# larrybb626/diffusion_models_dsdiff

Measured on AMD Instinct MI355X. Metric: 256x256 cDDPM slices/sec (1000-step), higher is better.
Workload: dtype f32 (operands split exactly into 3 bf16 pieces, 6 bf16-MFMA products, f32 accumulate)

## Files before the change

diffusion_models_dsdiff_amd/csrc/conv.hip:

```cpp
#include "device_common.h"

#include <string>

#include <cstdlib>

namespace dsd {

static constexpr size_t DIRECT_LDS_MAX = 128 * 1024;
static constexpr int BM = 128;
static constexpr int BK = 32;
static constexpr int LDS_STRIDE = 36;

struct ConvP {
    const float* x;
    const float* w;
    const float* bias;
    const float* emb;
    const float* res;
    float* y;
    int64_t x_bs;
    int N, H, W, Cin, Cout, OH, OW, ks, stride, pad, ups, emb_stride, out_nchw;
    int M, Ktot, cchunks, IHg, IWg, tiles_m, tiles_n, ohw;
    unsigned x_bytes, w_bytes;
    int y_ld;
// ... 215 lines not shown
    const int nwg = gridDim.x;
    int L = blockIdx.x;
    {
        const int cpx = nwg >> 3;
        if (L < (cpx << 3)) L = (L & 7) * cpx + (L >> 3);
    }
    const int tile_n = L % p.tiles_n;
    const int tile_m = L / p.tiles_n;
    const int m0 = tile_m * BM;
    const int n0 = tile_n * (NT * 32);

    const int col4 = tid & 7;
    const int srow = tid >> 3;
    int a_h[4], a_w[4];
    unsigned a_nb[4];
    bool a_ok[4];
#pragma unroll
    for (int i = 0; i < 4; ++i) {
        int m = m0 + srow + 32 * i;
        a_ok[i] = m < p.M;
        m = a_ok[i] ? m : 0;
        const int n = m / p.ohw;
        const int r = m - n * p.ohw;
        const int oh = r / p.OW;
        const int ow = r - oh * p.OW;
        a_h[i] = oh * p.stride - p.pad;
        a_w[i] = ow * p.stride - p.pad;
        a_nb[i] = (unsigned)n * (unsigned)p.x_bs + (unsigned)(col4 * 4);
    }
    unsigned b_voff[NT];
#pragma unroll
    for (int j = 0; j < NT; ++j) {
        const int n = n0 + srow + 32 * j;
        b_voff[j] = n < p.Cout ? ((unsigned)n * (unsigned)p.Ktot + (unsigned)(col4 * 4)) * 4u : OOB;
    }
    unsigned a_voff[4];
    auto tap_offsets = [&](int kh, int kw) {
#pragma unroll
        for (int i = 0; i < 4; ++i) {
            int ih = a_h[i] + kh, iw = a_w[i] + kw;
            const bool ok = a_ok[i] && (unsigned)ih < (unsigned)p.IHg && (unsigned)iw < (unsigned)p.IWg;
            if (p.ups) {
                ih >>= 1;
                iw >>= 1;
            }
            a_voff[i] = ok ? (a_nb[i] + (unsigned)(ih * p.W + iw) * (unsigned)p.Cin) * 4u : OOB;
        }
    };
    f32x4 ra[4], rb[NT];
    auto load_tile = [&](int soff_a, int soff_b) {
#pragma unroll
        for (int i = 0; i < 4; ++i) ra[i] = __builtin_bit_cast(f32x4, __builtin_amdgcn_raw_buffer_load_b128(rx, a_voff[i], soff_a, 0));
#pragma unroll
        for (int j = 0; j < NT; ++j) rb[j] = __builtin_bit_cast(f32x4, __builtin_amdgcn_raw_buffer_load_b128(rw, b_voff[j], soff_b, 0));
    };

    f32x16 acc[NT];
#pragma unroll
    for (int j = 0; j < NT; ++j)
#pragma unroll
        for (int r = 0; r < 16; ++r) acc[j][r] = 0.f;

    const int lrow = lane & 31;
    const int half = lane >> 5;
    const float* a_frag = As + (wave * 32 + lrow) * LDS_STRIDE + 4 * half;
    const float* b_frag = Bs + lrow * LDS_STRIDE + 4 * half;
    float* a_st = As + srow * LDS_STRIDE + col4 * 4;
    float* b_st = Bs + srow * LDS_STRIDE + col4 * 4;

    const int KT = p.ks * p.ks * p.cchunks;
    int kh = 0, kw = 0, cc = 0, tap = 0;
    tap_offsets(0, 0);
    load_tile(0, 0);
    for (int kt = 0; kt < KT; ++kt) {
        __syncthreads();
#pragma unroll
        for (int i = 0; i < 4; ++i) *reinterpret_cast<f32x4*>(a_st + 32 * i * LDS_STRIDE) = ra[i];
#pragma unroll
        for (int j = 0; j < NT; ++j) *reinterpret_cast<f32x4*>(b_st + 32 * j * LDS_STRIDE) = rb[j];
        __syncthreads();
        if (kt + 1 < KT) {
            if (++cc == p.cchunks) {
                cc = 0;
                ++tap;
                if (++kw == p.ks) {
                    kw = 0;
                    ++kh;
                }
                tap_offsets(kh, kw);
            }
            load_tile(cc * (BK * 4), (tap * p.Cin + cc * BK) * 4);
        }
        conv_tile_mfma<NT, 4, LDS_STRIDE>(a_frag, b_frag, acc);
    }
    conv_epilogue<NT>(p, acc, m0, n0, wave, lrow, half);
}

__global__ __launch_bounds__(256) void conv_direct_lds_kernel(ConvP p) {
    extern __shared__ float wl[];
    const int tid = threadIdx.x;
    for (int i = tid; i < p.Ktot * p.Cout; i += 256) {
        const int k = i / p.Cout, co = i - k * p.Cout;
        wl[i] = p.w[(int64_t)co * p.Ktot + k];
    }
    __syncthreads();
    const int c4n = p.Cout >> 2;
    const int PIX = 64;
    const int64_t pix0 = (int64_t)blockIdx.x * PIX;
    for (int idx = tid; idx < PIX * c4n; idx += 256) {
        const int pl = idx / c4n, c4 = idx - pl * c4n;
        const int64_t m = pix0 + pl;
        if (m >= p.M) break;
        const int nb = (int)(m / p.ohw);
        const int r = (int)(m - (int64_t)nb * p.ohw);
        const int oh = r / p.OW, ow = r - oh * p.OW;
        float4 acc = make_float4(0.f, 0.f, 0.f, 0.f);
        int k = 0;
        for (int kh = 0; kh < p.ks; ++kh)
            for (int kw = 0; kw < p.ks; ++kw) {
                int ih = oh * p.stride - p.pad + kh, iw = ow * p.stride - p.pad + kw;
                const bool ok = (unsigned)ih < (unsigned)p.IHg && (unsigned)iw < (unsigned)p.IWg;
                if (p.ups) {
                    ih >>= 1;
                    iw >>= 1;
                }
                const float* src = p.x + (int64_t)nb * p.x_bs + ((int64_t)ih * p.W + iw) * p.Cin;
                for (int ci = 0; ci < p.Cin; ++ci, ++k) {
                    const float xv = ok ? src[ci] : 0.f;
                    const float4 w4 = *reinterpret_cast<const float4*>(wl + k * p.Cout + c4 * 4);
                    acc.x = fmaf(xv, w4.x, acc.x);
                    acc.y = fmaf(xv, w4.y, acc.y);
                    acc.z = fmaf(xv, w4.z, acc.z);
                    acc.w = fmaf(xv, w4.w, acc.w);
                }
            }
        float v[4] = {acc.x, acc.y, acc.z, acc.w};
#pragma unroll
        for (int q = 0; q < 4; ++q) {
            const int n = c4 * 4 + q;
            if (p.bias) v[q] += p.bias[n];
            if (p.emb) v[q] += p.emb[(int64_t)nb * p.emb_stride + n];
            if (p.res) v[q] += p.res[m * p.Cout + n];
        }
        if (p.out_nchw) {
            for (int q = 0; q < 4; ++q) p.y[((int64_t)nb * p.Cout + c4 * 4 + q) * p.ohw + r] = v[q];
        } else {
            *reinterpret_cast<float4*>(p.y + m * p.y_ld + c4 * 4) = make_float4(v[0], v[1], v[2], v[3]);
        }
    }
}

template <int KMAX, bool STATS>
__global__ __launch_bounds__(256) void conv_direct_cols_kernel(ConvP p, int W4, int ppb, double* __restrict__ stats, int chunks) {
    __shared__ double sm[STATS ? 1024 : 1][2];
    const int rpi = blockDim.x / W4;
    const int row = threadIdx.x / W4;
    const int c4 = threadIdx.x - row * W4;
    double ss[4] = {0.0, 0.0, 0.0, 0.0}, qq[4] = {0.0, 0.0, 0.0, 0.0};
    float4 w[KMAX];
#pragma unroll
    for (int k = 0; k < KMAX; ++k) {
        if (k < p.Ktot) {
            w[k].x = p.w[(int64_t)(c4 * 4 + 0) * p.Ktot + k];
            w[k].y = p.w[(int64_t)(c4 * 4 + 1) * p.Ktot + k];
            w[k].z = p.w[(int64_t)(c4 * 4 + 2) * p.Ktot + k];
            w[k].w = p.w[(int64_t)(c4 * 4 + 3) * p.Ktot + k];
        } else {
            w[k] = make_float4(0.f, 0.f, 0.f, 0.f);
        }
    }
    int dh[KMAX], dw[KMAX], dc[KMAX];
#pragma unroll
    for (int k = 0; k < KMAX; ++k) {
        const int tap = k / p.Cin;
        dc[k] = k - tap * p.Cin;
        dh[k] = tap / p.ks - p.pad;
        dw[k] = tap - (tap / p.ks) * p.ks - p.pad;
    }
    const float4 b4 = p.bias ? *reinterpret_cast<const float4*>(p.bias + c4 * 4) : make_float4(0.f, 0.f, 0.f, 0.f);
    const int64_t m_end = min((int64_t)p.M, ((int64_t)blockIdx.x + 1) * ppb);
    int64_t m = (int64_t)blockIdx.x * ppb + row;
    int nb = (int)(m / p.ohw);
    int oh = (int)(m - (int64_t)nb * p.ohw) / p.OW;
    int ow = (int)(m - (int64_t)nb * p.ohw) - oh * p.OW;
    for (; m < m_end; m += rpi, ow += rpi) {
        while (ow >= p.OW) {
            ow -= p.OW;
            if (++oh == p.OH) {
                oh = 0;
                ++nb;
            }
        }
        float4 acc = make_float4(0.f, 0.f, 0.f, 0.f);
        const float* xb = p.x + (int64_t)nb * p.x_bs;
#pragma unroll
        for (int k = 0; k < KMAX; ++k) {
            int ih = oh * p.stride + dh[k], iw = ow * p.stride + dw[k];
            const bool ok = (k < p.Ktot) & ((unsigned)ih < (unsigned)p.IHg) & ((unsigned)iw < (unsigned)p.IWg);
            ih >>= p.ups;
            iw >>= p.ups;
            const float xv = ok ? xb[((int64_t)ih * p.W + iw) * p.Cin + dc[k]] : 0.f;
            acc.x = fmaf(xv, w[k].x, acc.x);
            acc.y = fmaf(xv, w[k].y, acc.y);
            acc.z = fmaf(xv, w[k].z, acc.z);
            acc.w = fmaf(xv, w[k].w, acc.w);
        }
        acc.x += b4.x; acc.y += b4.y; acc.z += b4.z; acc.w += b4.w;
        if (p.emb) {
            const float4 e = *reinterpret_cast<const float4*>(p.emb + (int64_t)nb * p.emb_stride + c4 * 4);
            acc.x += e.x; acc.y += e.y; acc.z += e.z; acc.w += e.w;
        }
        if (p.res) {
            const float4 e = *reinterpret_cast<const float4*>(p.res + m * p.Cout + c4 * 4);
            acc.x += e.x; acc.y += e.y; acc.z += e.z; acc.w += e.w;
        }
        *reinterpret_cast<float4*>(p.y + m * p.y_ld + c4 * 4) = acc;
        if (STATS) {
            const double a = acc.x, b = acc.y, c = acc.z, d = acc.w;
            ss[0] += a; qq[0] = fma(a, a, qq[0]);
            ss[1] += b; qq[1] = fma(b, b, qq[1]);
            ss[2] += c; qq[2] = fma(c, c, qq[2]);
            ss[3] += d; qq[3] = fma(d, d, qq[3]);
        }
    }
    if (STATS) {
        if (row > 0) {
#pragma unroll
            for (int e = 0; e < 4; ++e) {
                sm[row * p.Cout + c4 * 4 + e][0] = ss[e];
                sm[row * p.Cout + c4 * 4 + e][1] = qq[e];
            }
        }
        __syncthreads();
        if (row == 0) {
            for (int r = 1; r < rpi; ++r)
#pragma unroll
                for (int e = 0; e < 4; ++e) {
                    ss[e] += sm[r * p.Cout + c4 * 4 + e][0];
                    qq[e] += sm[r * p.Cout + c4 * 4 + e][1];
                }
            const int64_t m0 = (int64_t)blockIdx.x * ppb;
            const int n0 = (int)(m0 / p.ohw), chunk = (int)((m0 - (int64_t)n0 * p.ohw) / ppb);
            double* o = stats + (((int64_t)n0 * chunks + chunk) * p.Cout + c4 * 4) * 2;
#pragma unroll
            for (int e = 0; e < 4; ++e) {
                o[2 * e] = ss[e];
                o[2 * e + 1] = qq[e];
            }
        }
    }
}

__global__ __launch_bounds__(256) void conv_scalar_kernel(ConvP p) {
    const int64_t total = (int64_t)p.M * p.Cout;
    for (int64_t i = (int64_t)blockIdx.x * 256 + threadIdx.x; i < total; i += (int64_t)gridDim.x * 256) {
        const int64_t m = i / p.Cout;
        const int n = (int)(i - m * p.Cout);
        const int nb = (int)(m / p.ohw);
        const int r = (int)(m - (int64_t)nb * p.ohw);
        const int oh = r / p.OW, ow = r - oh * p.OW;
        float acc = 0.f;
        const float* wr = p.w + (int64_t)n * p.Ktot;
        for (int kh = 0; kh < p.ks; ++kh)
            for (int kw = 0; kw < p.ks; ++kw) {
                int ih = oh * p.stride - p.pad + kh, iw = ow * p.stride - p.pad + kw;
                if (!((unsigned)ih < (unsigned)p.IHg && (unsigned)iw < (unsigned)p.IWg)) continue;
                if (p.ups) {
                    ih >>= 1;
                    iw >>= 1;
                }
                const float* src = p.x + (int64_t)nb * p.x_bs + ((int64_t)ih * p.W + iw) * p.Cin;
                const float* wk = wr + (kh * p.ks + kw) * p.Cin;
                for (int ci = 0; ci < p.Cin; ++ci) acc = fmaf(src[ci], wk[ci], acc);
            }
        if (p.bias) acc += p.bias[n];
        if (p.emb) acc += p.emb[(int64_t)nb * p.emb_stride + n];
        if (p.res) acc += p.res[m * p.Cout + n];
        if (p.out_nchw)
            p.y[((int64_t)nb * p.Cout + n) * p.ohw + r] = acc;
        else
            p.y[m * p.y_ld + n] = acc;
    }
}

__global__ void pack_ohwi_kernel(const float* __restrict__ src, float* __restrict__ dst, int Cout, int Cin, int kk) {
    const int64_t total = (int64_t)Cout * Cin * kk;
    for (int64_t i = (int64_t)blockIdx.x * blockDim.x + threadIdx.x; i < total; i += (int64_t)gridDim.x * blockDim.x) {
        const int ci = (int)(i % Cin);
        const int64_t r = i / Cin;
        const int t = (int)(r % kk);
        const int co = (int)(r / kk);
        dst[i] = src[((int64_t)co * Cin + ci) * kk + t];
    }
}

void pack_ohwi(const float* w_oihw, float* w_ohwi, int Cout, int Cin, int ks, hipStream_t s) {
    const int64_t total = (int64_t)Cout * Cin * ks * ks;
    const int blocks = (int)std::min<int64_t>((total + 255) / 256, 65535);
    hipLaunchKernelGGL(pack_ohwi_kernel, dim3(blocks), dim3(256), 0, s, w_oihw, w_ohwi, Cout, Cin, ks * ks);
    check_launch("pack_ohwi");
}

double conv2d_flops(const ConvArgs& a) {
    int OH, OW;
    conv_out_hw(a, &OH, &OW);
    return 2.0 * a.N * OH * OW * (double)a.Cout * a.ks * a.ks * a.Cin;
}

double conv2d_exec_flops(const ConvArgs& a) { return a.w_subpixel ? conv2d_flops(a) * 4.0 / 9.0 : conv2d_flops(a); }

static int conv_variant(const ConvArgs& a) {
    if (a.variant >= 0) return a.variant;
    static const int env = [] {
        const char* e = getenv("DSD_CONV_VARIANT");
        return e ? atoi(e) : 0;
    }();
    return env;
}

static int pick_nt(int Cout, int tiles_m, int precision, int lanes = 1) {
    static const int force = [] {
        const char* e = getenv("DSD_FORCE_NT");
        return e ? atoi(e) : 0;
    }();
    if (force >= 1 && force <= 5) return force;
    const int t32 = cdiv(Cout, 32);
    const double t_fix = precision == PREC_F32 ? 500.0 : 700.0;
    const double t_mf = precision == PREC_F32 ? 1024.0 : (precision == PREC_BF16X6 ? 384.0 : 192.0);
    int best = 1;
    double best_t = 1e300;
    for (int nt = 5; nt >= 1; --nt) {
        const int64_t blocks = (int64_t)tiles_m * cdiv(t32, nt) * std::max(1, lanes);
        const double t = (double)cdiv(blocks, 512) * (t_fix + nt * t_mf);
        if (t < best_t * 0.999) {
            best_t = t;
            best = nt;
        }
    }
    return best;
}

static int direct_cols_ppb(const ConvArgs& a, int64_t M, int ohw, bool with_stats) {
    const int W4 = a.Cout / 4, rpi = 256 / W4;
    if (!with_stats) return std::max(rpi * 8, cdiv(cdiv(M, 8192), rpi) * rpi);
    for (int ppb = 128; ppb >= 16; ppb >>= 1)
        if (ohw % ppb == 0) return ppb;
    return 0;
}

ConvRoute conv2d_route(const ConvArgs& a, bool replan) {
    ConvRoute r;
    conv_out_hw(a, &r.OH, &r.OW);
    r.M = (int64_t)a.N * r.OH * r.OW;
    const int ohw = r.OH * r.OW, Ktot = a.ks * a.ks * a.Cin;
    r.precision = a.precision == PREC_F32 || !conv2d_split_eligible(a) ? PREC_F32 : a.precision;
    r.nt = pick_nt(a.Cout, cdiv(r.M, BM), r.precision, a.lanes);
    if (a.w_subpixel) {
        r.family = CONV_SUBPIXEL;
        r.precision = PREC_BF16X6;
        r.nt = 5;
        r.structure = 2;
        r.tap_reuse = true;
        r.stats_chunks = conv2d_subpixel_shape_ok(a) ? 4 * a.H * a.W / (2 * BM) : 0;
        return r;
    }
    if (a.Cin % 4 != 0 || Ktot < 32) {
        if (a.Cout % 4 == 0 && a.Cout / 4 <= 256 && Ktot <= 9 && !a.out_nchw && (!a.emb || a.emb_stride % 4 == 0)) {
            r.family = CONV_DIRECT_COLS;
            const int ppb = direct_cols_ppb(a, r.M, ohw, true);
            r.stats_chunks = ppb ? ohw / ppb : 0;
        } else {
            r.family = a.Cout % 4 == 0 && (size_t)Ktot * a.Cout * sizeof(float) <= DIRECT_LDS_MAX ? CONV_DIRECT_LDS : CONV_SCALAR;
        }
        return r;
    }
    if (r.precision == PREC_BF16X6 && conv2d_wino_eligible(a)) {
        r.family = CONV_WINO;
        r.stats_chunks = conv2d_wino_stats_chunks(a);
        return r;
    }
    if (r.precision == PREC_F32) {
        const int64_t x_bs = a.x_bs >= 0 ? a.x_bs : (int64_t)a.H * a.W * a.Cin;
        const int64_t xb = ((int64_t)(a.N - 1) * x_bs + (int64_t)a.H * a.W * a.Cin) * 4, wb = (int64_t)a.Cout * Ktot * 4;
        r.family = a.Cin % BK == 0 && xb < 0xFFFFFF00ll && wb < 0xFFFFFF00ll && conv_variant(a) == 0 ? CONV_MFMA_BUF : CONV_MFMA;
        return r;
    }
    r.family = CONV_SPLIT;
    int nt_p, ks_p, ad_p, nt_d, ks_d, ad_d;
    conv2d_split_plan(a, r.nt, &nt_p, &ks_p, &ad_p, true);
    conv2d_split_plan(a, r.nt, &nt_d, &ks_d, &ad_d, false);
    r.nt = replan ? nt_p : nt_d;
    r.ksplit = replan ? ks_p : ks_d;
    r.structure = replan ? ad_p : ad_d;
    r.launches = r.ksplit > 1 ? 2 : 1;
    r.scratch_bytes = r.ksplit > 1 ? (size_t)r.ksplit * r.M * a.Cout * sizeof(float) : 0;
// ... 99 lines not shown
```

diffusion_models_dsdiff_amd/csrc/norm.hip:

```cpp
#include "device_common.h"

#include <cstdlib>

namespace dsd {

static constexpr int GN_GROUPS = 32;

struct GnGeom {
    int threads;
    int k;
    int rpi;
    int ppc;
    int nchunk;
};

static GnGeom gn_geom(int HW, int C) {
    GnGeom g{};
    const int cols = C / 4;
    if (cols <= 256) {
        g.k = 1;
        g.rpi = 256 / cols;
        g.threads = g.rpi * cols;
    } else {
        g.k = 2;
        while (cols % g.k != 0 || cols / g.k > 256) ++g.k;
        g.rpi = 1;
        g.threads = cols / g.k;
    }
    int ppc = cdiv(HW, 256);
    if (ppc < 32) ppc = 32;
    ppc = cdiv(ppc, g.rpi) * g.rpi;
    g.ppc = ppc;
    g.nchunk = cdiv(HW, ppc);
    return g;
}

int gn_nchunks(int HW, int C) { return gn_geom(HW, C).nchunk; }

template <int K>
__global__ __launch_bounds__(256) void gn_stats_kernel(const float* __restrict__ x, int HW, int C, int rpi, int ppc,
                                                       double* __restrict__ partial) {
    extern __shared__ double sm[];
    const int cols = C >> 2;
    const int colsk = cols / K;
    const int tid = threadIdx.x;
    const int row = tid / colsk;
    const int col0 = tid - row * colsk;
    const int n = blockIdx.y, chunk = blockIdx.x;
    const int p0 = chunk * ppc;
    const int p1 = min(HW, p0 + ppc);
    double s[K][4], q[K][4];
#pragma unroll
    for (int k = 0; k < K; ++k)
#pragma unroll
        for (int e = 0; e < 4; ++e) s[k][e] = q[k][e] = 0.0;
    const float* base = x + (int64_t)n * HW * C;
    auto accum = [&](int k, const float4 v) {
        const double a = v.x, b = v.y, c = v.z, d = v.w;
        s[k][0] += a; q[k][0] = fma(a, a, q[k][0]);
        s[k][1] += b; q[k][1] = fma(b, b, q[k][1]);
        s[k][2] += c; q[k][2] = fma(c, c, q[k][2]);
        s[k][3] += d; q[k][3] = fma(d, d, q[k][3]);
    };
    int p = p0 + row;
    for (; p + 3 * rpi < p1; p += 4 * rpi) {
        float4 v[4][K];
#pragma unroll
        for (int u = 0; u < 4; ++u)
#pragma unroll
            for (int k = 0; k < K; ++k)
                v[u][k] = reinterpret_cast<const float4*>(base + (int64_t)(p + u * rpi) * C)[col0 + k * colsk];
#pragma unroll
        for (int u = 0; u < 4; ++u)
#pragma unroll
            for (int k = 0; k < K; ++k) accum(k, v[u][k]);
    }
    for (; p < p1; p += rpi) {
        const float4* rp = reinterpret_cast<const float4*>(base + (int64_t)p * C);
#pragma unroll
        for (int k = 0; k < K; ++k) accum(k, rp[col0 + k * colsk]);
    }
#pragma unroll
    for (int k = 0; k < K; ++k)
#pragma unroll
        for (int e = 0; e < 4; ++e) {
            const int c = (col0 + k * colsk) * 4 + e;
            sm[((int64_t)row * C + c) * 2 + 0] = s[k][e];
            sm[((int64_t)row * C + c) * 2 + 1] = q[k][e];
        }
    __syncthreads();
    for (int c = tid; c < C; c += blockDim.x) {
        double ss = 0.0, qq = 0.0;
        for (int r = 0; r < rpi; ++r) {
            ss += sm[((int64_t)r * C + c) * 2 + 0];
            qq += sm[((int64_t)r * C + c) * 2 + 1];
        }
        double* o = partial + (((int64_t)n * gridDim.x + chunk) * C + c) * 2;
        o[0] = ss;
        o[1] = qq;
    }
}

void gn_stats(const float* x, int N, int HW, int C, double* partial, int nchunk, hipStream_t s) {
    DSD_CHECK(C % GN_GROUPS == 0 && C % 4 == 0, "GroupNorm32: C=%d must be a multiple of 32", C);
    const GnGeom g = gn_geom(HW, C);
    DSD_CHECK(g.nchunk == nchunk, "gn_stats: chunk count mismatch");
    const size_t lds = (size_t)g.rpi * C * 2 * sizeof(double);
    DSD_CHECK(lds <= 64 * 1024, "gn_stats: C=%d too large", C);
    const dim3 grid(g.nchunk, N), block(g.threads);
    switch (g.k) {
        case 1: hipLaunchKernelGGL(gn_stats_kernel<1>, grid, block, lds, s, x, HW, C, g.rpi, g.ppc, partial); break;
        case 2: hipLaunchKernelGGL(gn_stats_kernel<2>, grid, block, lds, s, x, HW, C, g.rpi, g.ppc, partial); break;
        case 3: hipLaunchKernelGGL(gn_stats_kernel<3>, grid, block, lds, s, x, HW, C, g.rpi, g.ppc, partial); break;
        case 4: hipLaunchKernelGGL(gn_stats_kernel<4>, grid, block, lds, s, x, HW, C, g.rpi, g.ppc, partial); break;
        default: fail("gn_stats: C=%d needs %d columns per thread (unsupported)", C, g.k);
    }
    check_launch("gn_stats");
}

__global__ __launch_bounds__(256) void gn_finalize_kernel(GnSrc s0, GnSrc s1, int HW, int C,
                                                          const float* __restrict__ gamma,
                                                          const float* __restrict__ beta, float eps,
                                                          const float* __restrict__ film, int film_stride,
                                                          float* __restrict__ scale, float* __restrict__ shift) {
    __shared__ double red[256][2];
    __shared__ float mean_s, rstd_s;
    const int g = blockIdx.x, n = blockIdx.y, tid = threadIdx.x;
    const int cpg = C / GN_GROUPS;
    const int g0 = g * cpg, g1 = g0 + cpg;
    double ss = 0.0, qq = 0.0;
#pragma unroll
    for (int k = 0; k < 2; ++k) {
        const GnSrc& sr = k == 0 ? s0 : s1;
        if (!sr.p) continue;
        const int lo = max(g0, sr.c0), hi = min(g1, sr.c0 + sr.c);
        const int ncol = hi - lo;
        if (ncol <= 0) continue;
        const int items = sr.chunks * ncol;
        const double* base = sr.p + (int64_t)n * sr.chunks * sr.c * 2;
        for (int it = tid; it < items; it += 256) {
            const int ch = it / ncol, c = lo + (it - ch * ncol) - sr.c0;
            const double* o = base + ((int64_t)ch * sr.c + c) * 2;
            ss += o[0];
            qq += o[1];
        }
    }
    red[tid][0] = ss;
    red[tid][1] = qq;
    __syncthreads();
    for (int st = 128; st > 0; st >>= 1) {
        if (tid < st) {
            red[tid][0] += red[tid + st][0];
            red[tid][1] += red[tid + st][1];
        }
        __syncthreads();
    }
    if (tid == 0) {
        const double cnt = (double)HW * cpg;
        const double mean = red[0][0] / cnt;
        double var = red[0][1] / cnt - mean * mean;
        if (var < 0.0) var = 0.0;
        mean_s = (float)mean;
        rstd_s = (float)(1.0 / sqrt(var + (double)eps));
    }
    __syncthreads();
    for (int c = g0 + tid; c < g1; c += 256) {
        float sc = rstd_s * gamma[c];
        float sh = beta[c] - mean_s * sc;
        if (film) {
            const float f = 1.f + film[(int64_t)n * film_stride + c];
            sc *= f;
            sh = sh * f + film[(int64_t)n * film_stride + C + c];
        }
        scale[(int64_t)n * C + c] = sc;
        shift[(int64_t)n * C + c] = sh;
    }
}

void gn_finalize(const GnSrc& s0, const GnSrc& s1, int N, int HW, int C, const float* gamma, const float* beta,
                 float eps, const float* film, int film_stride, float* scale, float* shift, hipStream_t s) {
    DSD_CHECK(s0.p && s0.c0 == 0 && s0.c + (s1.p ? s1.c : 0) == C && (!s1.p || s1.c0 == s0.c),
              "gn_finalize: the statistic sources do not cover the %d channels", C);
    if (N == 0) return;
    hipLaunchKernelGGL(gn_finalize_kernel, dim3(GN_GROUPS, N), dim3(256), 0, s, s0, s1, HW, C, gamma, beta, eps, film,
                       film_stride, scale, shift);
    check_launch("gn_finalize");
}

template <int ACT, int V>
__global__ __launch_bounds__(256) void gn_small_kernel(const float* __restrict__ x, int HW, int C, const float* __restrict__ gamma,
                                                       const float* __restrict__ beta, float eps, const float* __restrict__ film,
                                                       int film_stride, float* __restrict__ y) {
    constexpr int U = 8;
    __shared__ double red[4][2];
    __shared__ float mean_s, rstd_s;
    const int g = blockIdx.x, n = blockIdx.y, tid = threadIdx.x, lane = tid & 63, wave = tid >> 6;
    const int cpg = C / GN_GROUPS, cv = cpg / V;
    const float* xb = x + (int64_t)n * HW * C + g * cpg;
    float* yb = y + (int64_t)n * HW * C + g * cpg;
    const int items = HW * cv;
    auto off = [&](int i) {
        const int p = i / cv, c = i - p * cv;
        return (int64_t)p * C + c * V;
    };
    double s = 0.0, q = 0.0;
    for (int i0 = tid; i0 < items; i0 += 256 * U) {
        float v[U][V];
#pragma unroll
        for (int u = 0; u < U; ++u) {
            const int i = i0 + u * 256;
#pragma unroll
            for (int k = 0; k < V; ++k) v[u][k] = 0.f;
            if (i < items) {
                if (V == 2) {
                    const float2 t = *reinterpret_cast<const float2*>(xb + off(i));
                    v[u][0] = t.x;
                    v[u][V - 1] = t.y;
                } else {
                    v[u][0] = xb[off(i)];
                }
            }
        }
#pragma unroll
        for (int u = 0; u < U; ++u)
#pragma unroll
            for (int k = 0; k < V; ++k) {
                const double d = v[u][k];
                s += d;
                q = fma(d, d, q);
            }
    }
    for (int o = 32; o > 0; o >>= 1) {
        s += __shfl_xor(s, o);
        q += __shfl_xor(q, o);
    }
    if (lane == 0) {
        red[wave][0] = s;
        red[wave][1] = q;
    }
    __syncthreads();
    if (tid == 0) {
        const double a = (red[0][0] + red[1][0]) + (red[2][0] + red[3][0]);
        const double b = (red[0][1] + red[1][1]) + (red[2][1] + red[3][1]);
        const double cnt = (double)HW * cpg;
        const double mean = a / cnt;
        double var = b / cnt - mean * mean;
        if (var < 0.0) var = 0.0;
        mean_s = (float)mean;
        rstd_s = (float)(1.0 / sqrt(var + (double)eps));
    }
    __syncthreads();
    const float mean = mean_s, rstd = rstd_s;
    auto coef = [&](int ch, float& sc, float& sh) {
        sc = rstd * gamma[ch];
        sh = beta[ch] - mean * sc;
        if (film) {
            const float f = 1.f + film[(int64_t)n * film_stride + ch];
            sc *= f;
            sh = sh * f + film[(int64_t)n * film_stride + C + ch];
        }
    };
    for (int i0 = tid; i0 < items; i0 += 256 * U) {
        float v[U][V];
#pragma unroll
        for (int u = 0; u < U; ++u) {
            const int i = i0 + u * 256;
            if (i < items) {
                if (V == 2) {
                    const float2 t = *reinterpret_cast<const float2*>(xb + off(i));
                    v[u][0] = t.x;
                    v[u][V - 1] = t.y;
                } else {
                    v[u][0] = xb[off(i)];
                }
            }
        }
#pragma unroll
        for (int u = 0; u < U; ++u) {
            const int i = i0 + u * 256;
            if (i >= items) continue;
            const int p = i / cv, c = (i - p * cv) * V;
            float o[V];
#pragma unroll
            for (int k = 0; k < V; ++k) {
                float sc, sh;
                coef(g * cpg + c + k, sc, sh);
                o[k] = fmaf(v[u][k], sc, sh);
                if (ACT == ACT_SILU) o[k] = silu_f(o[k]);
            }
            if (V == 2)
                *reinterpret_cast<float2*>(yb + (int64_t)p * C + c) = make_float2(o[0], o[V - 1]);
            else
                yb[(int64_t)p * C + c] = o[0];
        }
    }
}

bool gn_small_ok(int HW, int C) {
    static const bool on = getenv("DSD_GN_SMALL") != nullptr;
    return on && C % GN_GROUPS == 0 && (int64_t)HW * (C / GN_GROUPS) <= 32768;
}

void gn_small(const float* x, int N, int HW, int C, const float* gamma, const float* beta, float eps, const float* film,
              int film_stride, int act, float* y, hipStream_t s) {
    if ((int64_t)N * HW * C == 0) return;
    const bool v2 = (C / GN_GROUPS) % 2 == 0;
    const dim3 grid(GN_GROUPS, N), block(256);
#define DSD_GNS(A, VV) hipLaunchKernelGGL((gn_small_kernel<A, VV>), grid, block, 0, s, x, HW, C, gamma, beta, eps, film, film_stride, y)
    if (act == ACT_SILU) {
        if (v2) DSD_GNS(ACT_SILU, 2); else DSD_GNS(ACT_SILU, 1);
    } else {
        if (v2) DSD_GNS(ACT_NONE, 2); else DSD_GNS(ACT_NONE, 1);
    }
#undef DSD_GNS
    check_launch("gn_small");
}

template <int K, int ACT>
__global__ __launch_bounds__(256) void avg_stats_kernel(const float4* __restrict__ a, const float4* __restrict__ b,
                                                        const float4* __restrict__ c, const float4* __restrict__ d,
                                                        float div, int HW, int C, int rpi, int ppc, float* __restrict__ dst,
                                                        int dstC, int coff, int bmask, double* __restrict__ partial) {
    extern __shared__ double sm[];
    const int cols = C >> 2;
    const int colsk = cols / K;
    const int tid = threadIdx.x;
    const int row = tid / colsk;
    const int col0 = tid - row * colsk;
    const int n = blockIdx.y, chunk = blockIdx.x;
    const int p0 = chunk * ppc;
    const int p1 = min(HW, p0 + ppc);
    double s[K][4], q[K][4];
#pragma unroll
    for (int k = 0; k < K; ++k)
#pragma unroll
        for (int e = 0; e < 4; ++e) s[k][e] = q[k][e] = 0.0;
    const int64_t sb = (int64_t)n * HW * cols;
    for (int p = p0 + row; p < p1; p += rpi) {
#pragma unroll
        for (int k = 0; k < K; ++k) {
            const int c4 = col0 + k * colsk;
            const int64_t is = (int64_t)p * cols + c4, i = sb + is;
            float4 v = a[(bmask & 1) ? is : i];
            if (b) { const float4 t = b[(bmask & 2) ? is : i]; v.x += t.x; v.y += t.y; v.z += t.z; v.w += t.w; }
            if (c) { const float4 t = c[(bmask & 4) ? is : i]; v.x += t.x; v.y += t.y; v.z += t.z; v.w += t.w; }
            if (d) { const float4 t = d[(bmask & 8) ? is : i]; v.x += t.x; v.y += t.y; v.z += t.z; v.w += t.w; }
            if (div != 1.f) { v.x /= div; v.y /= div; v.z /= div; v.w /= div; }
            if (ACT == ACT_SILU) { v.x = silu_f(v.x); v.y = silu_f(v.y); v.z = silu_f(v.z); v.w = silu_f(v.w); }
            *reinterpret_cast<float4*>(dst + ((int64_t)n * HW + p) * dstC + coff + c4 * 4) = v;
            const double x0 = v.x, x1 = v.y, x2 = v.z, x3 = v.w;
            s[k][0] += x0; q[k][0] = fma(x0, x0, q[k][0]);
            s[k][1] += x1; q[k][1] = fma(x1, x1, q[k][1]);
            s[k][2] += x2; q[k][2] = fma(x2, x2, q[k][2]);
            s[k][3] += x3; q[k][3] = fma(x3, x3, q[k][3]);
        }
    }
#pragma unroll
    for (int k = 0; k < K; ++k)
#pragma unroll
        for (int e = 0; e < 4; ++e) {
            const int cc = (col0 + k * colsk) * 4 + e;
            sm[((int64_t)row * C + cc) * 2 + 0] = s[k][e];
            sm[((int64_t)row * C + cc) * 2 + 1] = q[k][e];
        }
    __syncthreads();
    for (int cc = tid; cc < C; cc += blockDim.x) {
        double ss = 0.0, qq = 0.0;
        for (int r = 0; r < rpi; ++r) {
            ss += sm[((int64_t)r * C + cc) * 2 + 0];
            qq += sm[((int64_t)r * C + cc) * 2 + 1];
        }
        double* o = partial + (((int64_t)n * gridDim.x + chunk) * C + cc) * 2;
        o[0] = ss;
        o[1] = qq;
    }
}

void avg_into_stats(const float* a, const float* b, const float* c, const float* d, float div, int N, int HW, int C,
                    float* dst, int dstC, int coff, int act, int bmask, double* partial, int nchunk, hipStream_t s) {
    DSD_CHECK(C % 4 == 0 && dstC % 4 == 0 && coff % 4 == 0, "avg_into_stats: channel counts must be multiples of 4");
    if ((int64_t)N * HW * C == 0) return;
    const GnGeom g = gn_geom(HW, C);
    DSD_CHECK(g.nchunk == nchunk, "avg_into_stats: chunk count mismatch");
    const size_t lds = (size_t)g.rpi * C * 2 * sizeof(double);
    DSD_CHECK(lds <= 64 * 1024, "avg_into_stats: C=%d too large", C);
    const dim3 grid(g.nchunk, N), block(g.threads);
#define DSD_AVG(KK)                                                                                                          \
    if (act == ACT_SILU)                                                                                                     \
        hipLaunchKernelGGL((avg_stats_kernel<KK, ACT_SILU>), grid, block, lds, s, (const float4*)a, (const float4*)b,        \
                           (const float4*)c, (const float4*)d, div, HW, C, g.rpi, g.ppc, dst, dstC, coff, bmask, partial);  \
    else                                                                                                                     \
        hipLaunchKernelGGL((avg_stats_kernel<KK, ACT_NONE>), grid, block, lds, s, (const float4*)a, (const float4*)b,        \
                           (const float4*)c, (const float4*)d, div, HW, C, g.rpi, g.ppc, dst, dstC, coff, bmask, partial);
    switch (g.k) {
        case 1: DSD_AVG(1) break;
        case 2: DSD_AVG(2) break;
        case 3: DSD_AVG(3) break;
        case 4: DSD_AVG(4) break;
        default: fail("avg_into_stats: C=%d needs %d columns per thread (unsupported)", C, g.k);
    }
#undef DSD_AVG
    check_launch("avg_into_stats");
}


template <int ACT>
__global__ __launch_bounds__(256) void affine_act_kernel(const float4* __restrict__ x, int HW, int cols, int W, int ppc,
                                                         const float4* __restrict__ scale, const float4* __restrict__ shift,
                                                         float4* __restrict__ y) {
    const int n = blockIdx.y;
    const int rpi = blockDim.x / W;
    const int row = threadIdx.x / W;
    const int cw = threadIdx.x - row * W;
    const int p0 = blockIdx.x * ppc;
    const int p1 = min(HW, p0 + ppc);
    const float4* xs = x + (int64_t)n * HW * cols;
    float4* ys = y + (int64_t)n * HW * cols;
    auto act = [](float4 v, const float4 sc, const float4 sh) {
        float4 o;
        o.x = fmaf(v.x, sc.x, sh.x);
        o.y = fmaf(v.y, sc.y, sh.y);
        o.z = fmaf(v.z, sc.z, sh.z);
        o.w = fmaf(v.w, sc.w, sh.w);
        if (ACT == ACT_SILU) {
            o.x = silu_f(o.x);
            o.y = silu_f(o.y);
            o.z = silu_f(o.z);
            o.w = silu_f(o.w);
        }
        return o;
    };
    for (int c4 = cw; c4 < cols; c4 += W) {
        const float4 sc = scale[(int64_t)n * cols + c4];
        const float4 sh = shift[(int64_t)n * cols + c4];
        int p = p0 + row;
        for (; p + 3 * rpi < p1; p += 4 * rpi) {
            const int64_t i0 = (int64_t)p * cols + c4, st = (int64_t)rpi * cols;
            const float4 v0 = xs[i0], v1 = xs[i0 + st], v2 = xs[i0 + 2 * st], v3 = xs[i0 + 3 * st];
            ys[i0] = act(v0, sc, sh);
            ys[i0 + st] = act(v1, sc, sh);
            ys[i0 + 2 * st] = act(v2, sc, sh);
            ys[i0 + 3 * st] = act(v3, sc, sh);
        }
        for (; p < p1; p += rpi) {
            const int64_t i0 = (int64_t)p * cols + c4;
            ys[i0] = act(xs[i0], sc, sh);
        }
    }
}

void affine_act(const float* x, int N, int HW, int C, const float* scale, const float* shift, int act, float* y,
                hipStream_t s) {
    const int cols = C / 4;
    if ((int64_t)N * HW * cols == 0) return;
    const int W = std::min(cols, 256);
    const int rpi = 256 / W, threads = rpi * W;
    int nchunk = std::max(1, std::min(4096 / std::max(N, 1), HW / (4 * rpi)));
    const int ppc = cdiv(cdiv(HW, nchunk), rpi) * rpi;
    nchunk = cdiv(HW, ppc);
    const dim3 grid((unsigned)nchunk, (unsigned)N);
    if (act == ACT_SILU)
        hipLaunchKernelGGL(affine_act_kernel<ACT_SILU>, grid, dim3(threads), 0, s, (const float4*)x, HW, cols, W, ppc,
                           (const float4*)scale, (const float4*)shift, (float4*)y);
    else
        hipLaunchKernelGGL(affine_act_kernel<ACT_NONE>, grid, dim3(threads), 0, s, (const float4*)x, HW, cols, W, ppc,
                           (const float4*)scale, (const float4*)shift, (float4*)y);
    check_launch("affine_act");
}

__global__ __launch_bounds__(256) void layer_norm_kernel(const float* __restrict__ x, int64_t rows, int C,
                                                         const float* __restrict__ gamma,
                                                         const float* __restrict__ beta, float eps,
                                                         float* __restrict__ y) {
    const int lane = threadIdx.x & 63;
    const int64_t row = (int64_t)blockIdx.x * 4 + (threadIdx.x >> 6);
    if (row >= rows) return;
    const float* xr = x + row * C;
    float s = 0.f;
    for (int c = lane; c < C; c += 64) s += xr[c];
    for (int o = 32; o > 0; o >>= 1) s += __shfl_xor(s, o);
    const float mean = s / C;
    float q = 0.f;
    for (int c = lane; c < C; c += 64) {
        const float d = xr[c] - mean;
        q = fmaf(d, d, q);
    }
    for (int o = 32; o > 0; o >>= 1) q += __shfl_xor(q, o);
    const float rstd = 1.f / sqrtf(q / C + eps);
    for (int c = lane; c < C; c += 64) y[row * C + c] = (xr[c] - mean) * rstd * gamma[c] + beta[c];
}

void layer_norm(const float* x, int64_t rows, int C, const float* gamma, const float* beta, float eps, float* y,
                hipStream_t s) {
    if (rows == 0) return;
    hipLaunchKernelGGL(layer_norm_kernel, dim3(cdiv(rows, 4)), dim3(256), 0, s, x, rows, C, gamma, beta, eps, y);
    check_launch("layer_norm");
}

}
```

Baseline: 0.04022.

## Stage conv inputs in LDS, vectorize GN stat reads, unroll avg-stats loads

The direct small-K conv kernel now has each thread gather one output pixel's input patch into shared memory, so the im2col gather happens once per pixel instead of once per output column group. All column threads then reuse the staged values, and the embedding load is cached per batch index. The stats scratch arrays move to a planar layout to cut LDS bank conflicts. GroupNorm finalize now reads partial sums as double2 with 4-way unrolling and reduces with wave shuffles instead of an LDS tree. avg_stats_kernel unrolls loads across pixels and sources and multiplies by an exact power-of-two reciprocal instead of dividing. These kernels are small or bandwidth-bound, the extra syncthreads and LDS use may lower occupancy, and the overall effect on a 1000-step run dominated by MFMA convs is likely small.

```diff
diff --git a/diffusion_models_dsdiff_amd/csrc/conv.hip b/diffusion_models_dsdiff_amd/csrc/conv.hip
--- a/diffusion_models_dsdiff_amd/csrc/conv.hip
+++ b/diffusion_models_dsdiff_amd/csrc/conv.hip
@@ -391,7 +391,9 @@
 
 template <int KMAX, bool STATS>
 __global__ __launch_bounds__(256) void conv_direct_cols_kernel(ConvP p, int W4, int ppb, double* __restrict__ stats, int chunks) {
-    __shared__ double sm[STATS ? 1024 : 1][2];
+    constexpr int XV = (KMAX + 1 + 3) / 4;
+    __shared__ uint4 xs[256 * XV];
+    __shared__ double sm[STATS ? 2048 : 1];
     const int rpi = blockDim.x / W4;
     const int row = threadIdx.x / W4;
     const int c4 = threadIdx.x - row * W4;
@@ -408,66 +410,88 @@
             w[k] = make_float4(0.f, 0.f, 0.f, 0.f);
         }
     }
-    int dh[KMAX], dw[KMAX], dc[KMAX];
-#pragma unroll
-    for (int k = 0; k < KMAX; ++k) {
-        const int tap = k / p.Cin;
-        dc[k] = k - tap * p.Cin;
-        dh[k] = tap / p.ks - p.pad;
-        dw[k] = tap - (tap / p.ks) * p.ks - p.pad;
-    }
     const float4 b4 = p.bias ? *reinterpret_cast<const float4*>(p.bias + c4 * 4) : make_float4(0.f, 0.f, 0.f, 0.f);
-    const int64_t m_end = min((int64_t)p.M, ((int64_t)blockIdx.x + 1) * ppb);
-    int64_t m = (int64_t)blockIdx.x * ppb + row;
-    int nb = (int)(m / p.ohw);
-    int oh = (int)(m - (int64_t)nb * p.ohw) / p.OW;
-    int ow = (int)(m - (int64_t)nb * p.ohw) - oh * p.OW;
-    for (; m < m_end; m += rpi, ow += rpi) {
-        while (ow >= p.OW) {
-            ow -= p.OW;
-            if (++oh == p.OH) {
-                oh = 0;
-                ++nb;
-            }
-        }
-        float4 acc = make_float4(0.f, 0.f, 0.f, 0.f);
-        const float* xb = p.x + (int64_t)nb * p.x_bs;
-#pragma unroll
-        for (int k = 0; k < KMAX; ++k) {
-            int ih = oh * p.stride + dh[k], iw = ow * p.stride + dw[k];
-            const bool ok = (k < p.Ktot) & ((unsigned)ih < (unsigned)p.IHg) & ((unsigned)iw < (unsigned)p.IWg);
-            ih >>= p.ups;
-            iw >>= p.ups;
-            const float xv = ok ? xb[((int64_t)ih * p.W + iw) * p.Cin + dc[k]] : 0.f;
-            acc.x = fmaf(xv, w[k].x, acc.x);
-            acc.y = fmaf(xv, w[k].y, acc.y);
-            acc.z = fmaf(xv, w[k].z, acc.z);
-            acc.w = fmaf(xv, w[k].w, acc.w);
-        }
-        acc.x += b4.x; acc.y += b4.y; acc.z += b4.z; acc.w += b4.w;
-        if (p.emb) {
-            const float4 e = *reinterpret_cast<const float4*>(p.emb + (int64_t)nb * p.emb_stride + c4 * 4);
-            acc.x += e.x; acc.y += e.y; acc.z += e.z; acc.w += e.w;
-        }
-        if (p.res) {
-            const float4 e = *reinterpret_cast<const float4*>(p.res + m * p.Cout + c4 * 4);
-            acc.x += e.x; acc.y += e.y; acc.z += e.z; acc.w += e.w;
-        }
-        *reinterpret_cast<float4*>(p.y + m * p.y_ld + c4 * 4) = acc;
-        if (STATS) {
-            const double a = acc.x, b = acc.y, c = acc.z, d = acc.w;
-            ss[0] += a; qq[0] = fma(a, a, qq[0]);
-            ss[1] += b; qq[1] = fma(b, b, qq[1]);
-            ss[2] += c; qq[2] = fma(c, c, qq[2]);
-            ss[3] += d; qq[3] = fma(d, d, qq[3]);
+    const int64_t m_begin = (int64_t)blockIdx.x * ppb;
+    const int64_t m_end = min((int64_t)p.M, m_begin + ppb);
+    const int T = blockDim.x;
+    float4 e4 = make_float4(0.f, 0.f, 0.f, 0.f);
+    int nb_e = -1;
+    for (int64_t mt = m_begin; mt < m_end; mt += T) {
+        const int tn = (int)min((int64_t)T, m_end - mt);
+        if (mt != m_begin) __syncthreads();
+        if (const int pl = threadIdx.x; pl < tn) {
+            const int m = (int)(mt + pl);
+            const int nb = m / p.ohw;
+            const int r = m - nb * p.ohw;
+            const int oh = r / p.OW, ow = r - oh * p.OW;
+            const float* xb = p.x + (int64_t)nb * p.x_bs;
+            unsigned t[XV * 4];
+#pragma unroll
+            for (int k = 0; k < XV * 4; ++k) t[k] = 0u;
+#pragma unroll
+            for (int k = 0; k < KMAX; ++k) {
+                if (k >= p.Ktot) break;
+                const int tap = k / p.Cin;
+                const int kh = tap / p.ks;
+                int ih = oh * p.stride + kh - p.pad, iw = ow * p.stride + (tap - kh * p.ks) - p.pad;
+                const bool ok = ((unsigned)ih < (unsigned)p.IHg) & ((unsigned)iw < (unsigned)p.IWg);
+                ih >>= p.ups;
+                iw >>= p.ups;
+                const float xv = ok ? xb[((int64_t)ih * p.W + iw) * p.Cin + (k - tap * p.Cin)] : 0.f;
+                t[k] = __float_as_uint(xv);
+            }
+            t[KMAX] = (unsigned)nb;
+#pragma unroll
+            for (int i = 0; i < XV; ++i) xs[pl * XV + i] = make_uint4(t[4 * i], t[4 * i + 1], t[4 * i + 2], t[4 * i + 3]);
+        }
+        __syncthreads();
+        for (int pl = row; pl < tn; pl += rpi) {
+            const int64_t m = mt + pl;
+            unsigned t[XV * 4];
+#pragma unroll
+            for (int i = 0; i < XV; ++i) {
+                const uint4 v = xs[pl * XV + i];
+                t[4 * i] = v.x; t[4 * i + 1] = v.y; t[4 * i + 2] = v.z; t[4 * i + 3] = v.w;
+            }
+            float4 acc = make_float4(0.f, 0.f, 0.f, 0.f);
+#pragma unroll
+            for (int k = 0; k < KMAX; ++k) {
+                const float xv = __uint_as_float(t[k]);
+                acc.x = fmaf(xv, w[k].x, acc.x);
+                acc.y = fmaf(xv, w[k].y, acc.y);
+                acc.z = fmaf(xv, w[k].z, acc.z);
+                acc.w = fmaf(xv, w[k].w, acc.w);
+            }
+            acc.x += b4.x; acc.y += b4.y; acc.z += b4.z; acc.w += b4.w;
+            if (p.emb) {
+                const int nb = (int)t[KMAX];
+                if (nb != nb_e) {
+                    e4 = *reinterpret_cast<const float4*>(p.emb + (int64_t)nb * p.emb_stride + c4 * 4);
+                    nb_e = nb;
+                }
+                acc.x += e4.x; acc.y += e4.y; acc.z += e4.z; acc.w += e4.w;
+            }
+            if (p.res) {
+                const float4 e = *reinterpret_cast<const float4*>(p.res + m * p.Cout + c4 * 4);
+                acc.x += e.x; acc.y += e.y; acc.z += e.z; acc.w += e.w;
+            }
+            *reinterpret_cast<float4*>(p.y + m * p.y_ld + c4 * 4) = acc;
+            if (STATS) {
+                const double a = acc.x, b = acc.y, c = acc.z, d = acc.w;
+                ss[0] += a; qq[0] = fma(a, a, qq[0]);
+                ss[1] += b; qq[1] = fma(b, b, qq[1]);
+                ss[2] += c; qq[2] = fma(c, c, qq[2]);
+                ss[3] += d; qq[3] = fma(d, d, qq[3]);
+            }
         }
     }
     if (STATS) {
+        const int plane = rpi * W4;
         if (row > 0) {
 #pragma unroll
             for (int e = 0; e < 4; ++e) {
-                sm[row * p.Cout + c4 * 4 + e][0] = ss[e];
-                sm[row * p.Cout + c4 * 4 + e][1] = qq[e];
+                sm[e * plane + row * W4 + c4] = ss[e];
+                sm[(4 + e) * plane + row * W4 + c4] = qq[e];
             }
         }
         __syncthreads();
@@ -475,11 +499,10 @@
             for (int r = 1; r < rpi; ++r)
 #pragma unroll
                 for (int e = 0; e < 4; ++e) {
-                    ss[e] += sm[r * p.Cout + c4 * 4 + e][0];
-                    qq[e] += sm[r * p.Cout + c4 * 4 + e][1];
-                }
-            const int64_t m0 = (int64_t)blockIdx.x * ppb;
-            const int n0 = (int)(m0 / p.ohw), chunk = (int)((m0 - (int64_t)n0 * p.ohw) / ppb);
+                    ss[e] += sm[e * plane + r * W4 + c4];
+                    qq[e] += sm[(4 + e) * plane + r * W4 + c4];
+                }
+            const int n0 = (int)(m_begin / p.ohw), chunk = (int)((m_begin - (int64_t)n0 * p.ohw) / ppb);
             double* o = stats + (((int64_t)n0 * chunks + chunk) * p.Cout + c4 * 4) * 2;
 #pragma unroll
             for (int e = 0; e < 4; ++e) {
diff --git a/diffusion_models_dsdiff_amd/csrc/norm.hip b/diffusion_models_dsdiff_amd/csrc/norm.hip
--- a/diffusion_models_dsdiff_amd/csrc/norm.hip
+++ b/diffusion_models_dsdiff_amd/csrc/norm.hip
@@ -1,6 +1,8 @@
 #include "device_common.h"
 
+#include <cmath>
 #include <cstdlib>
+#include <type_traits>
 
 namespace dsd {
 
@@ -123,8 +125,7 @@
                                                           const float* __restrict__ beta, float eps,
                                                           const float* __restrict__ film, int film_stride,
                                                           float* __restrict__ scale, float* __restrict__ shift) {
-    __shared__ double red[256][2];
-    __shared__ float mean_s, rstd_s;
+    __shared__ double red[2][256];
     const int g = blockIdx.x, n = blockIdx.y, tid = threadIdx.x;
     const int cpg = C / GN_GROUPS;
     const int g0 = g * cpg, g1 = g0 + cpg;
@@ -137,34 +138,60 @@
         const int ncol = hi - lo;
         if (ncol <= 0) continue;
         const int items = sr.chunks * ncol;
-        const double* base = sr.p + (int64_t)n * sr.chunks * sr.c * 2;
-        for (int it = tid; it < items; it += 256) {
-            const int ch = it / ncol, c = lo + (it - ch * ncol) - sr.c0;
-            const double* o = base + ((int64_t)ch * sr.c + c) * 2;
-            ss += o[0];
-            qq += o[1];
-        }
-    }
-    red[tid][0] = ss;
-    red[tid][1] = qq;
+        const double* base = sr.p + ((int64_t)n * sr.chunks * sr.c + (lo - sr.c0)) * 2;
+        const bool al16 = (reinterpret_cast<uintptr_t>(base) & 15) == 0;
+        const int qs = 256 / ncol, rs = 256 - qs * ncol;
+        int ch = tid / ncol, c = tid - ch * ncol;
+        const int64_t row2 = (int64_t)sr.c * 2;
+        auto load = [&](double2& v) {
+            const double* o = base + ch * row2 + c * 2;
+            if (al16) v = *reinterpret_cast<const double2*>(o);
+            else v = make_double2(o[0], o[1]);
+            ch += qs;
+            c += rs;
+            if (c >= ncol) {
+                c -= ncol;
+                ++ch;
+            }
+        };
+        int it = tid;
+        for (; it + 3 * 256 < items; it += 4 * 256) {
+            double2 v[4];
+#pragma unroll
+            for (int u = 0; u < 4; ++u) load(v[u]);
+#pragma unroll
+            for (int u = 0; u < 4; ++u) {
+                ss += v[u].x;
+                qq += v[u].y;
+            }
+        }
+        for (; it < items; it += 256) {
+            double2 v;
+            load(v);
+            ss += v.x;
+            qq += v.y;
+        }
+    }
+    red[0][tid] = ss;
+    red[1][tid] = qq;
     __syncthreads();
-    for (int st = 128; st > 0; st >>= 1) {
-        if (tid < st) {
-            red[tid][0] += red[tid + st][0];
-            red[tid][1] += red[tid + st][1];
-        }
-        __syncthreads();
-    }
-    if (tid == 0) {
-        const double cnt = (double)HW * cpg;
-        const double mean = red[0][0] / cnt;
-        double var = red[0][1] / cnt - mean * mean;
-        if (var < 0.0) var = 0.0;
-        mean_s = (float)mean;
-        rstd_s = (float)(1.0 / sqrt(var + (double)eps));
-    }
-    __syncthreads();
-    for (int c = g0 + tid; c < g1; c += 256) {
+    if (tid >= 64) return;
+    ss = (red[0][tid] + red[0][tid + 128]) + (red[0][tid + 64] + red[0][tid + 192]);
+    qq = (red[1][tid] + red[1][tid + 128]) + (red[1][tid + 64] + red[1][tid + 192]);
+#pragma unroll
+    for (int st = 32; st > 0; st >>= 1) {
+        ss += __shfl_down(ss, st);
+        qq += __shfl_down(qq, st);
+    }
+    ss = __shfl(ss, 0);
+    qq = __shfl(qq, 0);
+    const double cnt = (double)HW * cpg;
+    const double mean = ss / cnt;
+    double var = qq / cnt - mean * mean;
+    if (var < 0.0) var = 0.0;
+    const float mean_s = (float)mean;
+    const float rstd_s = (float)(1.0 / sqrt(var + (double)eps));
+    for (int c = g0 + tid; c < g1; c += 64) {
         float sc = rstd_s * gamma[c];
         float sh = beta[c] - mean_s * sc;
         if (film) {
@@ -319,9 +346,11 @@
 template <int K, int ACT>
 __global__ __launch_bounds__(256) void avg_stats_kernel(const float4* __restrict__ a, const float4* __restrict__ b,
                                                         const float4* __restrict__ c, const float4* __restrict__ d,
-                                                        float div, int HW, int C, int rpi, int ppc, float* __restrict__ dst,
-                                                        int dstC, int coff, int bmask, double* __restrict__ partial) {
+                                                        float div, float inv, int HW, int C, int rpi, int ppc,
+                                                        float* __restrict__ dst, int dstC, int coff, int bmask,
+                                                        double* __restrict__ partial) {
     extern __shared__ double sm[];
+    constexpr int U = K == 1 ? 4 : (K == 2 ? 2 : 1);
     const int cols = C >> 2;
     const int colsk = cols / K;
     const int tid = threadIdx.x;
@@ -336,41 +365,73 @@
 #pragma unroll
         for (int e = 0; e < 4; ++e) s[k][e] = q[k][e] = 0.0;
     const int64_t sb = (int64_t)n * HW * cols;
-    for (int p = p0 + row; p < p1; p += rpi) {
-#pragma unroll
-        for (int k = 0; k < K; ++k) {
-            const int c4 = col0 + k * colsk;
-            const int64_t is = (int64_t)p * cols + c4, i = sb + is;
-            float4 v = a[(bmask & 1) ? is : i];
-            if (b) { const float4 t = b[(bmask & 2) ? is : i]; v.x += t.x; v.y += t.y; v.z += t.z; v.w += t.w; }
-            if (c) { const float4 t = c[(bmask & 4) ? is : i]; v.x += t.x; v.y += t.y; v.z += t.z; v.w += t.w; }
-            if (d) { const float4 t = d[(bmask & 8) ? is : i]; v.x += t.x; v.y += t.y; v.z += t.z; v.w += t.w; }
-            if (div != 1.f) { v.x /= div; v.y /= div; v.z /= div; v.w /= div; }
-            if (ACT == ACT_SILU) { v.x = silu_f(v.x); v.y = silu_f(v.y); v.z = silu_f(v.z); v.w = silu_f(v.w); }
-            *reinterpret_cast<float4*>(dst + ((int64_t)n * HW + p) * dstC + coff + c4 * 4) = v;
-            const double x0 = v.x, x1 = v.y, x2 = v.z, x3 = v.w;
-            s[k][0] += x0; q[k][0] = fma(x0, x0, q[k][0]);
-            s[k][1] += x1; q[k][1] = fma(x1, x1, q[k][1]);
-            s[k][2] += x2; q[k][2] = fma(x2, x2, q[k][2]);
-            s[k][3] += x3; q[k][3] = fma(x3, x3, q[k][3]);
-        }
-    }
+    const float4* src[4] = {a, b, c, d};
+    int64_t so[4];
+#pragma unroll
+    for (int j = 0; j < 4; ++j) so[j] = ((bmask >> j) & 1) ? 0 : sb;
+    float* dcol = dst + (int64_t)n * HW * dstC + coff + col0 * 4;
+    auto finish = [&](int p, int k, float4 v) {
+        if (div != 1.f) {
+            if (inv != 0.f) { v.x *= inv; v.y *= inv; v.z *= inv; v.w *= inv; }
+            else { v.x /= div; v.y /= div; v.z /= div; v.w /= div; }
+        }
+        if (ACT == ACT_SILU) { v.x = silu_f(v.x); v.y = silu_f(v.y); v.z = silu_f(v.z); v.w = silu_f(v.w); }
+        *reinterpret_cast<float4*>(dcol + (int64_t)p * dstC + k * colsk * 4) = v;
+        const double x0 = v.x, x1 = v.y, x2 = v.z, x3 = v.w;
+        s[k][0] += x0; q[k][0] = fma(x0, x0, q[k][0]);
+        s[k][1] += x1; q[k][1] = fma(x1, x1, q[k][1]);
+        s[k][2] += x2; q[k][2] = fma(x2, x2, q[k][2]);
+        s[k][3] += x3; q[k][3] = fma(x3, x3, q[k][3]);
+    };
+    auto run = [&](auto ns) {
+        constexpr int NS = decltype(ns)::value;
+        auto trip = [&](int p, auto nu) {
+            constexpr int NU = decltype(nu)::value;
+            float4 v[NU][K][NS];
+#pragma unroll
+            for (int u = 0; u < NU; ++u)
+#pragma unroll
+                for (int k = 0; k < K; ++k) {
+                    const int64_t is = (int64_t)(p + u * rpi) * cols + col0 + k * colsk;
+#pragma unroll
+                    for (int j = 0; j < NS; ++j) v[u][k][j] = src[j][so[j] + is];
+                }
+#pragma unroll
+            for (int u = 0; u < NU; ++u)
+#pragma unroll
+                for (int k = 0; k < K; ++k) {
+                    float4 t = v[u][k][0];
+#pragma unroll
+                    for (int j = 1; j < NS; ++j) { t.x += v[u][k][j].x; t.y += v[u][k][j].y; t.z += v[u][k][j].z; t.w += v[u][k][j].w; }
+                    finish(p + u * rpi, k, t);
+                }
+        };
+        int p = p0 + row;
+        for (; p + (U - 1) * rpi < p1; p += U * rpi) trip(p, std::integral_constant<int, U>{});
+        for (; p < p1; p += rpi) trip(p, std::integral_constant<int, 1>{});
+    };
+    if (d) run(std::integral_constant<int, 4>{});
+    else if (c) run(std::integral_constant<int, 3>{});
+    else if (b) run(std::integral_constant<int, 2>{});
+    else run(std::integral_constant<int, 1>{});
+    const int plane = rpi * cols;
 #pragma unroll
     for (int k = 0; k < K; ++k)
 #pragma unroll
         for (int e = 0; e < 4; ++e) {
-            const int cc = (col0 + k * colsk) * 4 + e;
-            sm[((int64_t)row * C + cc) * 2 + 0] = s[k][e];
-            sm[((int64_t)row * C + cc) * 2 + 1] = q[k][e];
+            const int i = e * plane + row * cols + col0 + k * colsk;
+            sm[i] = s[k][e];
+            sm[4 * plane + i] = q[k][e];
         }
     __syncthreads();
-    for (int cc = tid; cc < C; cc += blockDim.x) {
+    for (int j = tid; j < C; j += blockDim.x) {
+        const int e = j / cols, col = j - e * cols;
         double ss = 0.0, qq = 0.0;
         for (int r = 0; r < rpi; ++r) {
-            ss += sm[((int64_t)r * C + cc) * 2 + 0];
-            qq += sm[((int64_t)r * C + cc) * 2 + 1];
-        }
-        double* o = partial + (((int64_t)n * gridDim.x + chunk) * C + cc) * 2;
+            ss += sm[e * plane + r * cols + col];
+            qq += sm[(4 + e) * plane + r * cols + col];
+        }
+        double* o = partial + (((int64_t)n * gridDim.x + chunk) * C + col * 4 + e) * 2;
         o[0] = ss;
         o[1] = qq;
     }
@@ -384,14 +445,17 @@
     DSD_CHECK(g.nchunk == nchunk, "avg_into_stats: chunk count mismatch");
     const size_t lds = (size_t)g.rpi * C * 2 * sizeof(double);
     DSD_CHECK(lds <= 64 * 1024, "avg_into_stats: C=%d too large", C);
+    DSD_CHECK((b || !c) && (c || !d), "avg_into_stats: sources are given in order (a, b, c, d)");
+    int ex = 0;
+    const float inv = std::frexp(div, &ex) == 0.5f && std::isnormal(1.f / div) ? 1.f / div : 0.f;
     const dim3 grid(g.nchunk, N), block(g.threads);
 #define DSD_AVG(KK)                                                                                                          \
     if (act == ACT_SILU)                                                                                                     \
         hipLaunchKernelGGL((avg_stats_kernel<KK, ACT_SILU>), grid, block, lds, s, (const float4*)a, (const float4*)b,        \
-                           (const float4*)c, (const float4*)d, div, HW, C, g.rpi, g.ppc, dst, dstC, coff, bmask, partial);  \
+                           (const float4*)c, (const float4*)d, div, inv, HW, C, g.rpi, g.ppc, dst, dstC, coff, bmask, partial);  \
     else                                                                                                                     \
         hipLaunchKernelGGL((avg_stats_kernel<KK, ACT_NONE>), grid, block, lds, s, (const float4*)a, (const float4*)b,        \
-                           (const float4*)c, (const float4*)d, div, HW, C, g.rpi, g.ppc, dst, dstC, coff, bmask, partial);
+                           (const float4*)c, (const float4*)d, div, inv, HW, C, g.rpi, g.ppc, dst, dstC, coff, bmask, partial);
     switch (g.k) {
         case 1: DSD_AVG(1) break;
         case 2: DSD_AVG(2) break;
```

Result: no change. 0.04039 (median of 6 runs) (+0.4%).
